# luntergroup/smcsmc

Hardware: AMD Instinct MI355X
Metric: genome segments/sec per EM iteration (Np=10000, 2 diploids, 100 Mb) (higher is better)
Workload: dtype f64

## Files before the change

profiles/stamps.py:

```python
import ctypes as C, os, sys, numpy as np, argparse
ROOT = os.path.dirname(os.path.dirname(os.path.abspath(__file__)))
sys.path.insert(0, ROOT)
from smcsmc_amd import pf, build as _build
ap = argparse.ArgumentParser(); ap.add_argument("--rows", type=int, default=6000); ap.add_argument("--debug", type=int, default=0)
ap.add_argument("--lib", default=None, help="a -DPF_STAMPS library built beforehand (default: build it, smcsmc_amd/build.py)")
a = ap.parse_args()
pf.LIB_PATH = a.lib or _build.build_stamps_lib()
import bench
args = argparse.Namespace(nsam=4, length=1e7, epochs=32, pops=1)
model, segs = bench.build_workload(args, seed=1)
f = pf.ParticleFilter(model, 10000, seed=1, max_trace_events=0, local_recomb=True, debug=a.debug)
f.load_segments(segs)
L = f.L
L.pf_debug_stamps.argtypes = [C.c_void_p, C.c_int64, C.c_void_p]; L.pf_debug_stamps.restype = C.c_int
f.init_prior(0.0); f.run(0, 200); f.sync()
rows = a.rows
assert L.pf_debug_stamps(f.h, rows, None) == 0
f.init_prior(0.0); f.run(0, rows); f.sync()
nc = (10000 + 63) // 64
out = np.zeros((rows, nc, 32), np.uint64)
assert L.pf_debug_stamps(f.h, rows, out.ctypes.data) == 0
st = out[5:, :, :9].astype(np.int64) * 10.0 / 1000.0
flag = f.trace()["resampled"][:rows]
t0 = st[:, :, 0].min(axis=1, keepdims=True)
rel = st - t0[:, :, None]
names = ["start", "loads issued", "decide_row done", "prologue done", "state ready", "update loop done", "site lik done", "stores issued", "scans done"]
end = rel[:, :, 8].max(axis=1)
print("rows", rows, "kernel span (first wave start -> last wave scans done): mean %.2f us" % end.mean())
for sel, nm in ((np.ones(len(end), bool), "all rows"), (flag[4:rows-1] == 1, "rows after a resampling row"), (flag[4:rows-1] == 0, "rows after a plain row")):
    sel = sel[:len(end)]
    print(nm, int(sel.sum()))
    for k in range(9):
        col = rel[sel][:, :, k]
        print("   %-18s mean over waves %6.2f   max over waves (mean over rows) %6.2f" % (names[k], col.mean(), col.max(axis=1).mean()))
    cr = rel[sel]
    idx = cr[:, :, 8].argmax(axis=1)
    crit = cr[np.arange(len(idx)), idx, :]
    print("   critical wave phase durations:", " ".join("%.2f" % v for v in np.diff(crit, axis=1).mean(axis=0)), " start offset %.2f" % crit[:, 0].mean())

sub = out[5:, :, 16:21].astype(np.int64) * 10.0 / 1000.0
selr = (flag[4:rows-1] == 1)[:len(end)]
if selr.any() and sub[selr].max() > 0:
    base = st[selr][:, :, 2]
    seq = [base] + [sub[selr][:, :, k] for k in range(5)] + [st[selr][:, :, 3]]
    nm = ["own offset (pipe_lo_from)", "search over wavefronts", "barrier, range, survivors", "staging decided, barrier", "search inside the wavefront", "first copy?, offspring table, barrier"]
    print("parent search, rows after a resampling row (mean over wavefronts of the step's duration):")
    for k in range(6):
        d = seq[k + 1] - seq[k]
        print("   %-40s %6.2f us" % (nm[k], d.mean()))

d = rel[:, :, 8] - rel[:, :, 4]
m = (len(d) // 2) * 2
pair = (d[0:m:2] + d[1:m:2]).max(axis=1)
single = d[0:m:2].max(axis=1) + d[1:m:2].max(axis=1)
pre = rel[:, :, 4].max(axis=1)
print("own work of a row (state ready -> scans done), slowest wavefront: %.2f us; two rows back to back, slowest wavefront: %.2f us per pair"
      " (two single rows: %.2f us); before it (launch start -> state ready, slowest wavefront): %.2f us" % (d.max(axis=1).mean(), pair.mean(), single.mean(), pre.mean()))
for k in (3, 4):
    mk = (len(d) // k) * k
    grp = sum(d[i:mk:k] for i in range(k)).max(axis=1)
    print("   %d rows back to back: %.2f us per group" % (k, grp.mean()))

acc = out[5:, :, 9:15].astype(np.int64)
trips = acc[:, :, 5].astype(float)
print("update trips per wave and row: mean %.2f, max over waves (mean over rows) %.2f" % (trips.mean(), trips.max(axis=1).mean()))
tot = acc[:, :, :5].sum(axis=(0, 1)) * 10.0 / 1000.0
names2 = ["no-mutation weight (all iterations)", "record head stores", "genealogy update", "record tail + tracked length", "next recombination position"]
for nm, v in zip(names2, tot):
    print("   %-40s %.3f us per trip" % (nm, v / max(1.0, trips.sum())))
acc2 = out[5:, :, 21:29].astype(np.int64)
tot2 = acc2.sum(axis=(0, 1)) * 10.0 / 1000.0
names3 = ["no-mutation weight: up to the factor (fastexp)", "no-mutation weight: the two products, loop control",
          "update: the four draws (table or Philox), next request", "update: cut point (slice, division, lineage)",
          "update: descendant mask", "update: node searches and intensities", "update: walk, inverse search, division",
          "update: tree edit (remove, slots, insert)"]
if tot2.sum() > 0:
    for nm, v in zip(names3, tot2):
        print("      %-52s %.3f us per trip" % (nm, v / max(1.0, trips.sum())))
    print("      %-52s %.3f us per trip" % ("update: tree length (rest of the slot)", (tot[2] - tot2[2:].sum()) / max(1.0, trips.sum())))
st_all = out[5:, :, :9].astype(np.int64) * 10.0 / 1000.0
ci = st_all[:, :, 8].argmax(axis=1)
ct = trips[np.arange(len(ci)), ci]
cl = (st_all[:, :, 5] - st_all[:, :, 4])[np.arange(len(ci)), ci]
print("wavefront that ends the launch: %.2f trips, %.2f us in the loop; wavefront with most trips: %.2f" % (ct.mean(), cl.mean(), trips.max(axis=1).mean()))
```

smcsmc_amd/csrc/pf_hip.hip:

```cpp
#include <hip/hip_runtime.h>
#include <type_traits>
#include <hip/hip_ext.h>

#include <algorithm>
#include <atomic>
#include <cmath>
#include <cstdio>
#include <cstdlib>
#include <cstring>
#include <string>
#include <vector>

#include "../../include/smcsmc_pf.h"
#include "pf_device.h"
#include "pf_types.h"
#include "pf_lane.h"
#include "pf_tree_reg.h"
#include "pf_lds_body.h"
#include "pf_mp_host.h"
#include "pf_wide_host.h"
#include "pf_pipe.h"
#include "pf_lds_pipe.h"

using namespace pf;

__global__ __launch_bounds__(PF_BS) void k_init(KArgs A, double initial_position) {
    extern __shared__ double smem[];
    init_lds_body(A, initial_position, smem);
}

__global__ __launch_bounds__(PF_BS) void k_extend(KArgs A, long long s) {
    extern __shared__ double smem[];
    extend_lds_body(A, s, smem);
}

__device__ __forceinline__ double in_vgpr(double x) { double y; asm("v_mov_b64 %0, %1" : "=v"(y) : "s"(x)); return y; }
__device__ __forceinline__ unsigned long long in_vgpr(unsigned long long x) { unsigned long long y; asm("v_mov_b64 %0, %1" : "=v"(y) : "s"(x)); return y; }

#ifdef PF_STAMPS
__device__ __forceinline__ void pf_acc_trip(unsigned long long* a) { a[5] += 1; }
#else
#define pf_acc_trip(a) do {} while (0)
#endif
#ifdef PF_STAMPS
#define PF_STAMP(k) do { if (A.stamps && (threadIdx.x & 63) == 0 && s < A.stamp_rows)                                   \
        A.stamps[((size_t)s * A.nc + (size_t)(((long long)pf_bx() * PF_BS + threadIdx.x) >> 6)) * PF_STAMP_W + (k)] = wall_clock64(); } while (0)
#define PF_TICK(var) unsigned long long var = wall_clock64()
#define PF_ACC(slot, t0, t1) pf_acc[slot] += (t1) - (t0)
#define PF_ACC_DECL unsigned long long pf_acc[6] = {0, 0, 0, 0, 0, 0}, pf_acc2[8] = {0, 0, 0, 0, 0, 0, 0, 0}
#define PF_ACC2(slot, t0, t1) pf_acc2[slot] += (t1) - (t0)
#define PF_ACC_STORE do { if (A.stamps && (threadIdx.x & 63) == 0 && s < A.stamp_rows) {                                \
        for (int k_ = 0; k_ < 6; ++k_)                                                                                  \
            A.stamps[((size_t)s * A.nc + (size_t)(((long long)pf_bx() * PF_BS + threadIdx.x) >> 6)) * PF_STAMP_W + 9 + k_] = pf_acc[k_]; \
        for (int k_ = 0; k_ < 8; ++k_)                                                                                  \
            A.stamps[((size_t)s * A.nc + (size_t)(((long long)pf_bx() * PF_BS + threadIdx.x) >> 6)) * PF_STAMP_W + 21 + k_] = pf_acc2[k_]; } } while (0)
#else
#define PF_STAMP(k) do {} while (0)
#define PF_TICK(var) do {} while (0)
#define PF_ACC(slot, t0, t1) do {} while (0)
#define PF_ACC2(slot, t0, t1) do {} while (0)
#define PF_ACC_DECL do {} while (0)
#define PF_ACC_STORE do {} while (0)
#endif

template <class KA>
__device__ __forceinline__ int gridDim_particles(const KA& A) { return (int)((A.Np + PF_BS - 1) / PF_BS); }

template <int NM, bool BIASED, bool EXACT = false, bool TREES = false, bool PIPE = false, class KA>
__device__ __forceinline__ void extend_reg_body(const KA& A, long long s, int fuse, PipeRow PR = PipeRow()) {
    extern __shared__ double smem[];
    double* sT = smem;
    double* sH = smem + PF_EPAD;
    double* sI = sH + PF_EPAD;
    double* sBH = sI + A.E;
    double* sBS = sBH + (PF_BIAS_MAX + 2);
    const Ctrl* c = A.ctrl;
    const int n = EXACT ? NM : A.n;
    const long long p = (long long)pf_bx() * PF_BS + threadIdx.x;
    const bool active = p < A.Np;
    const int lane = threadIdx.x & 63;
    PF_STAMP(0);
    RowPre pre;
    RTree<NM> t0;
    double o_wpost = 0.0, o_wpilot = 0.0, o_next = 0.0, o_xmark = 0.0, o_Ltree = 0.0, o_sm = 0.0, o_ebuf = 0.0;
    int o_ml = 0;
    unsigned o_widx = 0;
    unsigned long long o_ctr = 0;
    unsigned o_tab_end = 0;
    long long o_nres = 0; int o_bflag = 0, o_bgen = 0;
    double spec_sm[PF_PIPE_STAGE * 64 / PF_BS];
    int spec_lo = 0;
    double sg_start = 0.0, sg_len = 0.0;
    int sg_limit = 0, sg_state = 1;
    int sg_allele[NM];
#pragma unroll
    for (int i = 0; i < NM; ++i) sg_allele[i] = 0;
    if constexpr (PIPE) {
        if (PR.extend) {
            sg_start = A.seg_start[s]; sg_len = A.seg_len[s];
            sg_limit = A.seg_limit[s]; sg_state = A.seg_state[s];
            const int8_t* al = A.seg_alleles + (size_t)s * n;
#pragma unroll
            for (int i = 0; i < NM; ++i) if (i < n) sg_allele[i] = al[i];
        }
    }
    if constexpr (PIPE) {
        const int fs = __builtin_amdgcn_readfirstlane(PR.slot_prev >= 0 ? PR.slot_prev : c->cur);
        if (PR.complete) {
            pre = row_preload(A, fs);
            o_nres = c->xr[(fs + PF_RING - 1) & (PF_RING - 1)].n_res; o_bflag = c->xr[(fs + PF_RING - 1) & (PF_RING - 1)].flag; o_bgen = c->xr[(fs + PF_RING - 1) & (PF_RING - 1)].gen;
            spec_lo = pf_bx() * (PF_BS / 64) - (PF_PIPE_STAGE - PF_BS / 64) / 2;
            if (spec_lo > A.nc - PF_PIPE_STAGE) spec_lo = A.nc - PF_PIPE_STAGE;
            if (spec_lo < 0) spec_lo = 0;
            if (A.flags & 256) spec_lo = -0x40000000;
            const double* sm0 = A.rg_scan1m + (size_t)fs * A.Np;
#pragma unroll
            for (int k = 0; k < PF_PIPE_STAGE * 64 / PF_BS; ++k) {
                const long long src = (long long)spec_lo * 64 + k * PF_BS + threadIdx.x;
                spec_sm[k] = (src >= 0 && src < A.Np) ? sm0[src] : PF_INF;
            }
        }
        if (active) {
            const DState own = state_slot(A, fs);
#pragma unroll
            for (int r = 0; r < RTree<NM>::NI; ++r) {
                t0.S[r] = 0.0; t0.C0[r] = 0; t0.C1[r] = 0;
                if (r < n - 1) {
                    t0.S[r] = own.S[(size_t)r * A.Np + p];
                    t0.C0[r] = own.C[(size_t)(2 * r) * A.Np + p];
                    t0.C1[r] = own.C[(size_t)(2 * r + 1) * A.Np + p];
                }
            }
            o_wpost = own.w_post[p]; o_wpilot = own.w_pilot[p]; o_next = own.next_base[p]; o_xmark = own.x_mark[p];
            o_ml = own.mark_limit[p]; o_Ltree = own.Ltree[p];
            o_widx = PR.complete ? A.rg_widx[(size_t)fs * A.Np + p] : A.widx[p];
            o_ctr = A.rng_ctr[p]; o_ebuf = A.ebuf[p];
            if (PR.draws) o_tab_end = (unsigned)A.dt_filled[(size_t)((PR.draws - 1) ^ 1) * A.Np + p];
            if (PR.complete) o_sm = A.rg_scan1m[(size_t)fs * A.Np + p];
        }
    }
    for (int e = threadIdx.x; e < PF_EPAD; e += blockDim.x) {
        sT[e] = e < A.E ? A.T[e] : PF_INF;
        sH[e] = e < A.E ? A.Hc[e] : PF_INF;
        if (e < A.E) sI[e] = A.inv2N[e];
    }
    if (BIASED && threadIdx.x < PF_BIAS_MAX + 2) {
        sBH[threadIdx.x] = A.bias_H[threadIdx.x];
        if (threadIdx.x < PF_BIAS_MAX + 1) sBS[threadIdx.x] = A.bias_S[threadIdx.x];
    }
    __shared__ unsigned s_lut[PIPE ? 2 * PF_LUT_N / 4 : 1];
    const bool use_lut = PIPE && A.lut != nullptr;
    if constexpr (PIPE) {
        if (use_lut && threadIdx.x < 2 * PF_LUT_N / 4) s_lut[threadIdx.x] = ((const unsigned*)A.lut)[threadIdx.x];
    }
    int cur = 0, from_slot = 0;
    bool completing = false, gather = false;
    double inv = 1.0, S1v = 0.0, pos_prev = 0.0;
    int lo_p = 0, lo_p1 = 0;
    bool first_copy = true;
    long long a = p;
    int G_end = 0, ev = 0;
    if constexpr (PIPE) {
        PipeLds q = pipe_carve(sBS + (PF_BIAS_MAX + 1), A.nc);
        cur = PR.slot_out; from_slot = PR.slot_prev >= 0 ? PR.slot_prev : c->cur;
        completing = PR.complete != 0;
        pos_prev = PR.pos_prev;
        if (completing) {
            const int row_slot = from_slot;
            const long long n_res = o_nres + o_bflag;
            G_end = o_bgen + o_bflag;
            ev = (int)n_res;
            PF_STAMP(1);
#pragma unroll
            for (int k = 0; k < PF_PIPE_STAGE * 64 / PF_BS; ++k) q.stage[k * PF_BS + threadIdx.x] = spec_sm[k];
            RowDecision d = decide_row<true>(A, q, row_slot, n_res, pre);
            PF_STAMP(2);
            inv = d.inv; S1v = d.S1;
            gather = d.flag != 0;
            if (pf_bx() == 0 && threadIdx.x == 0) {
                Ctrl* cw = A.ctrl;
                cw->xr[row_slot].n_res = n_res; cw->xr[row_slot].gen = G_end; cw->xr[row_slot].flag = d.flag;
            }
            if (gather) {
                const double dn = (double)A.Np;
                const double invS1 = 1.0 / d.S1;
                const double* sm = A.rg_scan1m + (size_t)row_slot * A.Np;
                const int wave = threadIdx.x >> 6;
                int ch_own = (int)(p >> 6);
                double coff_own = 0.0, v_own = 0.0;
                int lo_next = 0;
                if (active) {
                    coff_own = pipe_chunk_offset(q, ch_own);
                    double w = coff_own + o_sm;
                    v_own = q.pmx[ch_own] > w ? q.pmx[ch_own] : w;
                    lo_next = p + 1 < A.Np ? pipe_lo_from(v_own, dn, A.Np, d.S1, invS1, d.u) : (int)A.Np;
                    q.slo[threadIdx.x] = lo_next;
                }
                PF_STAMP(16);
                const double lhs = ((double)p + d.u) * d.S1;
                int pch = 0;
                if (active) {
                    int lo_c = 0, hi_c = A.nc - 1;
                    while (lo_c < hi_c) {
                        int mid = (lo_c + hi_c) >> 1;
                        if (lhs < dn * q.pmx[mid + 1]) hi_c = mid; else lo_c = mid + 1;
                    }
                    pch = lo_c;
                }
                PF_STAMP(17);
                int cmin = active ? pch : 0x7fffffff, cmax = active ? pch : -1;
#pragma unroll
                for (int m = 1; m < 64; m <<= 1) {
                    int o1 = __shfl_xor(cmin, m, 64), o2 = __shfl_xor(cmax, m, 64);
                    cmin = o1 < cmin ? o1 : cmin; cmax = o2 > cmax ? o2 : cmax;
                }
                if (lane == 0) { q.wint[wave] = cmin; q.wint[PF_BS / 64 + wave] = cmax; }
                __syncthreads();
                if (active) lo_p1 = lo_next;
                if (active) {
                    if (threadIdx.x > 0) lo_p = q.slo[threadIdx.x - 1];
                    else lo_p = p > 0 ? pipe_lo_from(q.pmx[ch_own], dn, A.Np, d.S1, invS1, d.u) : 0;
                }
                cmin = q.wint[0]; cmax = q.wint[PF_BS / 64];
                for (int w = 1; w < PF_BS / 64; ++w) {
                    cmin = q.wint[w] < cmin ? q.wint[w] : cmin;
                    cmax = q.wint[PF_BS / 64 + w] > cmax ? q.wint[PF_BS / 64 + w] : cmax;
                }
                {
                    unsigned long long bal = __ballot(active && lo_p1 > lo_p);
                    if (lane == 0) q.wint[2 * (PF_BS / 64) + wave] = __popcll(bal);
                }
                PF_STAMP(18);
                int nst = cmax - cmin + 1;
                if (nst > PF_PIPE_STAGE) nst = PF_PIPE_STAGE;
                if (nst < 0) nst = 0;
                int stage_lo = cmin;
                if (cmin >= spec_lo && cmax < spec_lo + PF_PIPE_STAGE) {
                    stage_lo = spec_lo; nst = PF_PIPE_STAGE;
                } else {
                    __syncthreads();
                    for (int idx = threadIdx.x; idx < nst * 64; idx += PF_BS) {
                        long long src = (long long)cmin * 64 + idx;
                        q.stage[idx] = src < A.Np ? sm[src] : PF_INF;
                    }
                }
                __syncthreads();
                PF_STAMP(19);
                if (threadIdx.x == 0) {
                    int tot = 0;
                    for (int w = 0; w < PF_BS / 64; ++w) tot += q.wint[2 * (PF_BS / 64) + w];
                    A.rg_blkcnt[(size_t)row_slot * gridDim_particles(A) * A.blk_gran + pf_bx()] = tot;
                }
                if (active) {
                    const double coff_p = pipe_chunk_offset(q, pch);
                    const double pm_p = q.pmx[pch];
                    const bool staged = pch >= stage_lo && pch - stage_lo < nst;
                    auto val_at = [&](int l) -> double {
                        long long idx = (long long)pch * 64 + l;
                        double smv = staged ? q.stage[(pch - stage_lo) * 64 + l] : (idx < A.Np ? sm[idx] : PF_INF);
                        double w = coff_p + smv;
                        return pm_p > w ? pm_p : w;
                    };
                    int lo_l = 0, hi_l = 63;
                    while (lo_l < hi_l) {
                        int mid = (lo_l + hi_l) >> 1;
                        if (lhs < dn * val_at(mid)) hi_l = mid; else lo_l = mid + 1;
                    }
                    a = (long long)pch * 64 + lo_l;
                    PF_STAMP(20);
                    if (a > A.Np - 1) a = A.Np - 1;
                    const int la = (int)(a & 63);
                    if (p == 0 || a == 0) first_copy = (p == 0);
                    else {
                        double vprev = la > 0 ? val_at(la - 1) : pm_p;
                        if (a != (long long)pch * 64 + lo_l) {
                            long long am = a - 1;
                            int chm = (int)(am >> 6);
                            double w = pipe_chunk_offset(q, chm) + sm[am];
                            vprev = q.pmx[chm] > w ? q.pmx[chm] : w;
                        }
                        first_copy = ((((double)(p - 1)) + d.u) * d.S1 < dn * vprev);
                    }
                    int* lo_tab = A.lo + (size_t)(G_end % A.Gcap) * (A.Np + 1);
                    lo_tab[p] = lo_p;
                    if (p == A.Np - 1) lo_tab[A.Np] = (int)A.Np;
                }
            }
        }
    } else {
        cur = c->cur;
        completing = fuse != 0;
        gather = fuse && c->flag;
        from_slot = gather ? (cur ^ 1) : cur;
        __syncthreads();
    }
    if constexpr (PIPE) __syncthreads();
    PF_STAMP(3);
    cur = __builtin_amdgcn_readfirstlane(cur);
    from_slot = __builtin_amdgcn_readfirstlane(from_slot);
    double w_post = 0.0, w_pilot = 0.0;
    bool has_pending = false;
    if (active) {
        const DState st = state_slot(A, cur);
        const DState from = state_slot(A, from_slot);
        if constexpr (!PIPE) {
            a = gather ? (long long)A.parent[p] : p;
            const int* lo_tab = A.lo + (size_t)((c->gen - 1 + A.Gcap) % A.Gcap) * (A.Np + 1);
            if (gather) { lo_p = lo_tab[p]; lo_p1 = lo_tab[p + 1]; first_copy = (p == lo_tab[a]); }
            inv = c->inv_T; S1v = c->S1; pos_prev = c->cur_pos;
            G_end = c->gen - 1; ev = (int)c->n_resample - 1;
        }
        RTree<NM> t;
        const bool reload = !PIPE || gather;
        if (!reload) t = t0;
        else {
#pragma unroll
            for (int r = 0; r < RTree<NM>::NI; ++r) {
                t.S[r] = 0.0; t.C0[r] = 0; t.C1[r] = 0;
                if (r < n - 1) {
                    t.S[r] = from.S[(size_t)r * A.Np + a];
                    t.C0[r] = from.C[(size_t)(2 * r) * A.Np + a];
                    t.C1[r] = from.C[(size_t)(2 * r + 1) * A.Np + a];
                }
            }
        }
        RCtx cx;
        const double v_L = in_vgpr(A.L), v_mu = in_vgpr(A.mu), v_rho = in_vgpr(A.rho);
        cx.T = sT; cx.I = sI; cx.H = sH; cx.E = A.E; cx.n = n; cx.L = v_L; cx.mu = v_mu; cx.rho = v_rho;
        cx.seed = in_vgpr(A.seed); cx.slot = (unsigned)p; cx.stream = 0;
        cx.nb = A.n_bias + 1; cx.bH = sBH; cx.bS = sBS; cx.last_iw = 1.0;
        cx.want_desc = A.lmap_opp != nullptr || TREES; cx.want_desc_new = TREES; cx.last_desc = 0; cx.last_desc_new = 0;
        cx.vbc = A.vb_coal; cx.upd_fac = 1.0;
        cx.gK = BIASED ? A.g_K : 0; cx.gpos = A.g_pos; cx.grho = A.g_rho; cx.gleaf = A.g_leaf; cx.last_rbiw = 1.0;
        cx.ridx = cx.gK > 0 ? from.ridx[a] : 0; cx.g_rp = 0; cx.g_sb = 0;
        if constexpr (PIPE) {
            cx.lutT = use_lut ? (const unsigned char*)s_lut : nullptr;
            cx.lutH = use_lut ? (const unsigned char*)s_lut + PF_LUT_N : nullptr;
            cx.kbT = A.lut_kbT; cx.kbH = A.lut_kbH;
            cx.tab = nullptr; cx.tab_end = 0; cx.pf_ok = false; cx.pf_ctr = 0; cx.draws_log = false;
            if (PR.draws) {
                cx.tab = (const double2*)A.dt_tab + (size_t)p * PF_DRAW_RING;
                cx.tab_end = o_tab_end;
            }
        }
        DStore ds;
        if (BIASED) {
            d_bind(ds, A, st, p);
            ds.count = from.dcount[a]; ds.total = from.total_delayed[a];
            if (gather || PIPE)
                for (int k = 0; k < ds.count; ++k) {
                    st.dpos[(size_t)k * A.Np + p] = from.dpos[(size_t)k * A.Np + a];
                    st.dfac[(size_t)k * A.Np + p] = from.dfac[(size_t)k * A.Np + a];
                    st.ddelta[(size_t)k * A.Np + p] = from.ddelta[(size_t)k * A.Np + a];
                    st.dk[(size_t)k * A.Np + p] = from.dk[(size_t)k * A.Np + a];
                }
        }
        double next_base, x_mark;
        int mark_limit;
        unsigned widx;
        if (reload) {
            w_post = from.w_post[a];
            w_pilot = from.w_pilot[a];
            next_base = from.next_base[a];
            x_mark = from.x_mark[a];
            mark_limit = from.mark_limit[a];
            cx.Ltree = from.Ltree[a];
        } else {
            w_post = o_wpost; w_pilot = o_wpilot; next_base = o_next; x_mark = o_xmark; mark_limit = o_ml; cx.Ltree = o_Ltree;
        }
        if constexpr (PIPE) { cx.ctr = o_ctr; cx.ebuf = o_ebuf; widx = o_widx; r_draws_prefetch(cx); }
        else { cx.ctr = A.rng_ctr[p]; cx.ebuf = A.ebuf[p]; widx = A.widx[p]; }
        if (completing) {
            if (!PIPE && p == 0) { Ctrl* cw = A.ctrl; cw->gen_prev = c->gen; cw->nres_prev = c->n_resample; }
            if (!gather) {
                w_post *= inv;
                w_pilot *= inv;
            } else {
                const int G = G_end;
                const double pos = pos_prev;
                const DState& src = from;
                if (lo_p1 > lo_p) {
                    double* rec = rec_ptr(A, p, widx);
                    rec[0] = PIPE ? o_xmark : src.x_mark[p];
                    rec[1] = pos;
                    rec[2] = 0.0; rec[3] = 0.0;
                    rec[4] = __longlong_as_double((long long)make_meta(1, PIPE ? o_ml : src.mark_limit[p], -1, n));
                    if constexpr (PIPE) {
#pragma unroll
                        for (int r = 0; r < RTree<NM>::NI; ++r) if (r < n - 1) rec[5 + r] = t0.S[r];
                    } else {
                        for (int r = 0; r < n - 1; ++r) rec[5 + r] = src.S[(size_t)r * A.Np + p];
                    }
                    ++widx;
                }
                A.gstart[(size_t)((G + 1) % A.Gcap) * A.Np + p] = widx;
                if (ev < A.max_trace_events) A.ev_parents[(size_t)ev * A.Np + p] = (int)a;
                double wp = w_post * inv;
                double wq = w_pilot * inv;
                double sumn = S1v * inv;
                double adj = sumn / ((double)A.Np * wq);
                w_post = wp * adj;
                w_pilot = wq * adj;
                x_mark = pos;
                if (!first_copy && pos < v_L) {
                    next_base = r_sample_next_base<false>(cx, pos);
                    if constexpr (PIPE) r_draws_prefetch(cx);
                }
            }
        }

        PF_STAMP(4);
        const bool do_extend = !PIPE || PR.extend != 0;
        const int8_t* data = A.seg_alleles + (size_t)s * n;
        double seg_end = 0.0;
        int limit = 0;
        if constexpr (PIPE) { if (do_extend) { seg_end = sg_start + sg_len; limit = sg_limit; } }
        else { if (do_extend) { seg_end = A.seg_start[s] + A.seg_len[s]; limit = A.seg_limit[s]; } }
        const double extend_to = seg_end < v_L ? seg_end : v_L;
        unsigned one_mask = 0, zero_mask = 0, present_mask = 0, two_mask = 0;
        int missing = 0;
        if (do_extend)
#pragma unroll
            for (int i = 0; i < NM; ++i) if (i < n) {
                int d = PIPE ? sg_allele[i] : (int)data[i];
                missing += d == -1;
                if (d == 1) one_mask |= 1u << i;
                if (d == 0) zero_mask |= 1u << i;
                if (d == 2) two_mask |= 1u << i;
                if (d >= 0) present_mask |= 1u << i;
            }
        int leaf_status = 0;
        if (missing == 0) leaf_status = 1;
        if (missing == n) leaf_status = -1;

        double updated_to = (PIPE && completing) ? pos_prev : c->cur_pos;
        if (!do_extend) updated_to = extend_to;
        double B;
        if (leaf_status == -1) B = 0;
        else if (leaf_status == 1) B = cx.Ltree;
        else B = r_tracked_len(t, n, present_mask);

        PF_ACC_DECL;
        while (updated_to < extend_to) {
            PF_TICK(tk0);
            double new_to = extend_to < next_base ? extend_to : next_base;
            double f = fastexp(-v_mu * B * (new_to - updated_to));
            PF_TICK(tk0a);
            PF_ACC2(0, tk0, tk0a);
            w_post *= f;
            w_pilot *= f;
            if (BIASED && cx.gK > 0) {
                double dist = new_to - updated_to;
                double target_rate = dist * v_rho * cx.Ltree;
                double sampled_rate = dist * cx.grho[cx.ridx] * cx.Ltree;
                double iws = fastexp(sampled_rate - target_rate);
                w_post *= iws;
                w_pilot *= iws;
            }
            updated_to = new_to;
            if (BIASED && cx.gK > 0 && updated_to < extend_to && cx.ridx + 1 < cx.gK && updated_to == cx.gpos[cx.ridx + 1]) {
                cx.ridx += 1;
                next_base = r_sample_next_base<false>(cx, updated_to);
                if constexpr (PIPE) r_draws_prefetch(cx);
                continue;
            }
            PF_TICK(tk1);
            PF_ACC(0, tk0, tk1);
            PF_ACC2(1, tk0a, tk1);
            if (updated_to < extend_to) {
                double* rec = rec_ptr(A, p, widx);
                rec[0] = x_mark;
                rec[1] = updated_to;
#pragma unroll
                for (int r = 0; r < RTree<NM>::NI; ++r) if (r < n - 1) rec[5 + r] = t.S[r];
                double h, tc;
                PF_TICK(tk2);
                PF_ACC(1, tk1, tk2);
                r_genealogy_update<NM, BIASED, PIPE, PIPE && EXACT && NM == 4 && !BIASED && !TREES>(cx, t, &h, &tc);
                PF_TICK(tk3);
                PF_ACC(2, tk2, tk3);
#ifdef PF_STAMPS
                PF_ACC2(2, tk2, cx.gt[0]);
                for (int k_ = 0; k_ < 5; ++k_) PF_ACC2(3 + k_, cx.gt[k_], cx.gt[k_ + 1]);
#endif
                if (cx.vbc) { w_post *= cx.upd_fac; w_pilot *= cx.upd_fac; cx.upd_fac = 1.0; }
                rec[2] = h;
                rec[3] = tc;
                rec[4] = __longlong_as_double((long long)make_meta(0, mark_limit, limit, n, cx.last_desc, TREES ? cx.last_desc_new : 0u));
                ++widx;
                if (leaf_status == 0) B = r_tracked_len(t, n, present_mask);
                if (leaf_status == 1) B = cx.Ltree;
                PF_TICK(tk4);
                PF_ACC(3, tk3, tk4);
                pf_acc_trip(pf_acc);
                if (BIASED) {
                    double iw = cx.last_iw, rbiw = cx.last_rbiw;
                    double delay_height = (A.delay_type & 3) == 0 ? h : tc;
                    int idx = 0;
                    while (idx + 1 < cx.nb + 1 && sBH[idx + 1] < delay_height) ++idx;
                    if (idx >= cx.nb) idx = cx.nb - 1;
                    if (sBS[idx] == 1.0 && !(A.delay_type & 4)) { w_post *= rbiw; w_pilot *= rbiw; iw /= rbiw; }
                    double delay = A.app_delays[r_epoch_of(cx, delay_height)];
                    d_adjust_with_delay(ds, w_post, w_pilot, iw, delay, updated_to);
                }
                PF_TICK(tk5);
                next_base = r_sample_next_base<true, PIPE>(cx, updated_to);
                x_mark = updated_to;
                mark_limit = limit;
                PF_TICK(tk6);
                PF_ACC(4, tk5, tk6);
            }
        }
        PF_ACC_STORE;

        PF_STAMP(5);
        const KA& A1 = pf_reopen(A);
        const DState st1 = state_slot(A1, cur);
        if (BIASED) {
            for (;;) {
                if (ds.count == 0 || !do_extend) break;
                double pm = ds.pos[0];
                for (int i = 1; i < ds.count; ++i) { double pi = ds.pos[(size_t)i * ds.Np]; if (pi < pm) pm = pi; }
                if (!(pm < extend_to)) break;
                d_apply_earliest(ds, w_pilot);
            }
            st1.dcount[p] = ds.count;
            st1.total_delayed[p] = ds.total;
            if (cx.gK > 0) st1.ridx[p] = cx.ridx;
            has_pending = ds.count > 0;
        }
        if (do_extend && (PIPE ? sg_state : (int)A1.seg_state[s]) == 0) {
            const bool dephase = A1.flags & 2;
            const bool anc = A1.flags & 1;
            unsigned het_pairs = 0;
            int ncfg = 1;
            for (int i = 0; i + 1 < n; i += 2) {
                bool d0_two = (two_mask >> i) & 1u;
                bool one0 = (one_mask >> i) & 1u, one1 = (one_mask >> (i + 1)) & 1u;
                bool zero0 = (zero_mask >> i) & 1u, zero1 = (zero_mask >> (i + 1)) & 1u;
                bool het = d0_two || (dephase && ((one0 && zero1) || (zero0 && one1)));
                if (het) {
                    ncfg *= 2;
                    het_pairs |= 1u << i;
                    one_mask &= ~(3u << i); zero_mask &= ~(3u << i);
                    zero_mask |= 1u << i;
                    one_mask |= 1u << (i + 1);
                }
            }
            double norm = 1.0 / (double)ncfg;
            RBranchP<NM> bprob;
            r_site_branch_probs(t, n, v_mu, bprob);
            double lik = 0;
            for (;;) {
                lik += r_site_lik_from(t, n, bprob, one_mask, zero_mask, anc);
                if (ncfg == 1) break;
                bool more = false;
                for (int i = 0; i + 1 < n; i += 2) {
                    if (!((het_pairs >> i) & 1)) continue;
                    if ((zero_mask >> i) & 1) {
                        zero_mask &= ~(1u << i); one_mask |= 1u << i;
                        one_mask &= ~(1u << (i + 1)); zero_mask |= 1u << (i + 1);
                        more = true;
                        break;
                    }
                    one_mask &= ~(1u << i); zero_mask |= 1u << i;
                    zero_mask &= ~(1u << (i + 1)); one_mask |= 1u << (i + 1);
                }
                if (!more) break;
            }
            lik *= norm;
            w_post *= lik;
            w_pilot *= lik;
        }

        PF_STAMP(6);
#pragma unroll
        for (int r = 0; r < RTree<NM>::NI; ++r)
            if (r < n - 1) {
                st1.S[(size_t)r * A1.Np + p] = t.S[r];
                st1.C[(size_t)(2 * r) * A1.Np + p] = (int8_t)t.C0[r];
                st1.C[(size_t)(2 * r + 1) * A1.Np + p] = (int8_t)t.C1[r];
            }
        st1.w_post[p] = w_post;
        st1.w_pilot[p] = w_pilot;
        st1.next_base[p] = next_base;
        st1.x_mark[p] = x_mark;
        st1.mark_limit[p] = mark_limit;
        st1.Ltree[p] = cx.Ltree;
        A1.rng_ctr[p] = cx.ctr;
        A1.ebuf[p] = cx.ebuf;
        if constexpr (PIPE) {
            if (PR.draws) A1.dt_ctr[(size_t)(PR.draws - 1) * A1.Np + p] = cx.ctr;
            A1.rg_widx[(size_t)cur * A1.Np + p] = widx;
            if (!do_extend) A1.widx[p] = widx;
            if (PR.ahead) {
                const unsigned kold = A1.gstart[(size_t)(A1.ctrl->g_safe % A1.Gcap) * A1.Np + p];
                if (widx - kold > A1.cap && !A1.ctrl->err) A1.ctrl->err = ERR_LOG_OVERFLOW;
            }
        } else {
            A1.widx[p] = widx;
        }
        if (TREES && widx >= A1.cap) A1.ctrl->err = ERR_LOG_OVERFLOW;
        if constexpr (!PIPE) {
#pragma unroll
            for (int r = 0; r < RTree<NM>::NI; ++r) if (r < n - 1) A1.snap_S[A1.sp][(size_t)r * A1.Np + p] = t.S[r];
            A1.snap_w[A1.sp][p] = w_post; A1.snap_xm[A1.sp][p] = x_mark; A1.snap_ml[A1.sp][p] = mark_limit; A1.snap_widx[A1.sp][p] = widx;
        }
    }
    PF_STAMP(7);
    const KA& A2 = pf_reopen(A);
    double sp = wave_tree_sum(w_post);
    double sq = wave_tree_sum(w_pilot * w_pilot);
    double sc = wave_hs_scan(w_pilot, lane);
    double scp = wave_hs_scan(w_post, lane);
    double scm = wave_max_scan_d(sc, lane);
    long long chunk = p >> 6;
    PF_STAMP(8);
    if constexpr (PIPE) {
        const size_t ro = (size_t)cur * A2.Np, co = (size_t)cur * A2.nc;
        if (active) { A2.rg_scan1[ro + p] = sc; A2.rg_scanp[ro + p] = scp; A2.rg_scan1m[ro + p] = scm; }
        if (p == A2.Np - 1) A2.ctrl->last1[cur] = sc;
        if (lane == 63 && chunk < A2.nc) {
            A2.rg_cpost[co + chunk] = sp;
            A2.rg_csq[co + chunk] = sq;
            A2.rg_cpil[co + chunk] = sc;
            A2.rg_cpp[co + chunk] = scp;
            A2.rg_cmx1[co + chunk] = scm;
        }
        if (BIASED) {
            unsigned long long pend = __ballot(has_pending);
            if (lane == 0 && chunk < A2.nc) {
                A2.rg_dpend[co + chunk] = __popcll(pend);
                if (!PR.extend) A2.chunk_dpend[chunk] = __popcll(pend);
            }
        }
    } else {
        if (active) { A2.scan1[p] = sc; A2.scanp2[A2.sp][p] = scp; A2.scan1m[p] = scm; }
        if (lane == 63 && chunk < (A2.Np + 63) / 64) {
            A2.chunk_post[chunk] = sp;
            A2.chunk_sq[chunk] = sq;
            A2.chunk_pil[chunk] = sc;
            A2.chunk_pp[chunk] = scp;
            A2.chunk_mx1[chunk] = scm;
        }
        if (BIASED) {
            unsigned long long pend = __ballot(has_pending);
            if (lane == 0 && chunk < (A2.Np + 63) / 64) A2.chunk_dpend[chunk] = __popcll(pend);
        }
    }
}

template <int NM, bool BIASED, bool TREES = false>
__global__ __launch_bounds__(PF_BS) void k_extend_reg(KArgs A, long long s, int fuse) {
    extend_reg_body<NM, BIASED, false, TREES>(A, s, fuse);
}

#define PF_FIN_TILE_B 64
#define PF_FIN_PAIRS 64

template <class KA>
__device__ void finalize_counts(const KA& A, Ctrl* c, int tid, int nthreads, double* stage ) {
    const int E = A.E;
    const int nb = A.nbx;
// ... 3770 lines not shown
```

Baseline: 40210.

## Issue parent state loads early in resampling prologue, drop cross-wave staging

After: 40280, median of 4. No clear change (+0.2%).

```diff
diff --git a/profiles/stamps.py b/profiles/stamps.py
--- a/profiles/stamps.py
+++ b/profiles/stamps.py
@@ -43,11 +43,14 @@
 if selr.any() and sub[selr].max() > 0:
     base = st[selr][:, :, 2]
     seq = [base] + [sub[selr][:, :, k] for k in range(5)] + [st[selr][:, :, 3]]
-    nm = ["own offset (pipe_lo_from)", "search over wavefronts", "barrier, range, survivors", "staging decided, barrier", "search inside the wavefront", "first copy?, offspring table, barrier"]
-    print("parent search, rows after a resampling row (mean over wavefronts of the step's duration):")
+    nm = ["search over wavefronts", "search inside the wavefront", "parent's state requested, own offset (pipe_lo_from)",
+          "barrier, offsets exchanged, survivors", "first copy?, offspring table", "barrier, survivor sum"]
+    print("prologue, rows after a resampling row (mean over wavefronts of the step's duration):")
     for k in range(6):
         d = seq[k + 1] - seq[k]
-        print("   %-40s %6.2f us" % (nm[k], d.mean()))
+        print("   %-52s %6.2f us" % (nm[k], d.mean()))
+    far = out[5:, :, 29].astype(np.int64)[selr]
+    print("   lanes that read the scans from memory: %.3f %% of the lanes of these rows (%d rows with any)" % (100.0 * far.sum() / (selr.sum() * 10000.0), int((far.sum(axis=1) > 0).sum())))
 
 d = rel[:, :, 8] - rel[:, :, 4]
 m = (len(d) // 2) * 2
diff --git a/smcsmc_amd/csrc/pf_hip.hip b/smcsmc_amd/csrc/pf_hip.hip
--- a/smcsmc_amd/csrc/pf_hip.hip
+++ b/smcsmc_amd/csrc/pf_hip.hip
@@ -36,6 +36,12 @@
 
 __device__ __forceinline__ double in_vgpr(double x) { double y; asm("v_mov_b64 %0, %1" : "=v"(y) : "s"(x)); return y; }
 __device__ __forceinline__ unsigned long long in_vgpr(unsigned long long x) { unsigned long long y; asm("v_mov_b64 %0, %1" : "=v"(y) : "s"(x)); return y; }
+
+__device__ __forceinline__ void pf_lds_barrier() {
+    __builtin_amdgcn_fence(__ATOMIC_RELEASE, "workgroup", "local");
+    __builtin_amdgcn_s_barrier();
+    __builtin_amdgcn_fence(__ATOMIC_ACQUIRE, "workgroup", "local");
+}
 
 #ifdef PF_STAMPS
 __device__ __forceinline__ void pf_acc_trip(unsigned long long* a) { a[5] += 1; }
@@ -160,6 +166,9 @@
     bool first_copy = true;
     long long a = p;
     int G_end = 0, ev = 0;
+    RTree<NM> tpar;
+    double pa_wpost = 0.0, pa_wpilot = 0.0, pa_next = 0.0, pa_xmark = 0.0, pa_Ltree = 0.0, pa_total = 0.0;
+    int pa_ml = 0, pa_ridx = 0, pa_dcount = 0;
     if constexpr (PIPE) {
         PipeLds q = pipe_carve(sBS + (PF_BIAS_MAX + 1), A.nc);
         cur = PR.slot_out; from_slot = PR.slot_prev >= 0 ? PR.slot_prev : c->cur;
@@ -186,17 +195,6 @@
                 const double invS1 = 1.0 / d.S1;
                 const double* sm = A.rg_scan1m + (size_t)row_slot * A.Np;
                 const int wave = threadIdx.x >> 6;
-                int ch_own = (int)(p >> 6);
-                double coff_own = 0.0, v_own = 0.0;
-                int lo_next = 0;
-                if (active) {
-                    coff_own = pipe_chunk_offset(q, ch_own);
-                    double w = coff_own + o_sm;
-                    v_own = q.pmx[ch_own] > w ? q.pmx[ch_own] : w;
-                    lo_next = p + 1 < A.Np ? pipe_lo_from(v_own, dn, A.Np, d.S1, invS1, d.u) : (int)A.Np;
-                    q.slo[threadIdx.x] = lo_next;
-                }
-                PF_STAMP(16);
                 const double lhs = ((double)p + d.u) * d.S1;
                 int pch = 0;
                 if (active) {
@@ -207,68 +205,75 @@
                     }
                     pch = lo_c;
                 }
+                PF_STAMP(16);
+                const double coff_p = pipe_chunk_offset(q, pch);
+                const double pm_p = q.pmx[pch];
+                const bool staged = pch >= spec_lo && pch - spec_lo < PF_PIPE_STAGE;
+                auto val_at = [&](int l) -> double {
+                    long long idx = (long long)pch * 64 + l;
+                    double smv = q.stage[(staged ? (pch - spec_lo) * 64 : 0) + l];
+                    if (!staged) { smv = idx < A.Np ? sm[idx] : PF_INF; asm volatile("" : "+v"(smv)); }
+                    double w = coff_p + smv;
+                    return pm_p > w ? pm_p : w;
+                };
+                int lo_l = 0;
+                if (active) {
+                    int hi_l = 63;
+                    while (lo_l < hi_l) {
+                        int mid = (lo_l + hi_l) >> 1;
+                        if (lhs < dn * val_at(mid)) hi_l = mid; else lo_l = mid + 1;
+                    }
+                    a = (long long)pch * 64 + lo_l;
+                    if (a > A.Np - 1) a = A.Np - 1;
+                }
                 PF_STAMP(17);
-                int cmin = active ? pch : 0x7fffffff, cmax = active ? pch : -1;
+#ifdef PF_STAMPS
+                {
+                    const unsigned long long far = __ballot(active && !staged);
+                    if (A.stamps && lane == 0 && s < A.stamp_rows)
+                        A.stamps[((size_t)s * A.nc + (size_t)(((long long)pf_bx() * PF_BS + threadIdx.x) >> 6)) * PF_STAMP_W + 29] = __popcll(far);
+                }
+#endif
+                if (active) {
+                    const DState from = state_slot(A, __builtin_amdgcn_readfirstlane(row_slot));
 #pragma unroll
-                for (int m = 1; m < 64; m <<= 1) {
-                    int o1 = __shfl_xor(cmin, m, 64), o2 = __shfl_xor(cmax, m, 64);
-                    cmin = o1 < cmin ? o1 : cmin; cmax = o2 > cmax ? o2 : cmax;
+                    for (int r = 0; r < RTree<NM>::NI; ++r) {
+                        tpar.S[r] = 0.0; tpar.C0[r] = 0; tpar.C1[r] = 0;
+                        if (r < n - 1) {
+                            tpar.S[r] = from.S[(size_t)r * A.Np + a];
+                            tpar.C0[r] = from.C[(size_t)(2 * r) * A.Np + a];
+                            tpar.C1[r] = from.C[(size_t)(2 * r + 1) * A.Np + a];
+                        }
+                    }
+                    pa_wpost = from.w_post[a]; pa_wpilot = from.w_pilot[a]; pa_next = from.next_base[a]; pa_xmark = from.x_mark[a];
+                    pa_ml = from.mark_limit[a]; pa_Ltree = from.Ltree[a];
+                    if (BIASED) {
+                        if (A.g_K > 0) pa_ridx = from.ridx[a];
+                        pa_dcount = from.dcount[a]; pa_total = from.total_delayed[a];
+                    }
                 }
-                if (lane == 0) { q.wint[wave] = cmin; q.wint[PF_BS / 64 + wave] = cmax; }
-                __syncthreads();
+                const int ch_own = (int)(p >> 6);
+                int lo_next = 0;
+                if (active) {
+                    const double coff_own = pipe_chunk_offset(q, ch_own);
+                    double w = coff_own + o_sm;
+                    const double v_own = q.pmx[ch_own] > w ? q.pmx[ch_own] : w;
+                    lo_next = p + 1 < A.Np ? pipe_lo_from(v_own, dn, A.Np, d.S1, invS1, d.u) : (int)A.Np;
+                    q.slo[threadIdx.x] = lo_next;
+                }
+                PF_STAMP(18);
+                pf_lds_barrier();
                 if (active) lo_p1 = lo_next;
                 if (active) {
                     if (threadIdx.x > 0) lo_p = q.slo[threadIdx.x - 1];
                     else lo_p = p > 0 ? pipe_lo_from(q.pmx[ch_own], dn, A.Np, d.S1, invS1, d.u) : 0;
                 }
-                cmin = q.wint[0]; cmax = q.wint[PF_BS / 64];
-                for (int w = 1; w < PF_BS / 64; ++w) {
-                    cmin = q.wint[w] < cmin ? q.wint[w] : cmin;
-                    cmax = q.wint[PF_BS / 64 + w] > cmax ? q.wint[PF_BS / 64 + w] : cmax;
-                }
                 {
                     unsigned long long bal = __ballot(active && lo_p1 > lo_p);
-                    if (lane == 0) q.wint[2 * (PF_BS / 64) + wave] = __popcll(bal);
+                    if (lane == 0) q.wint[wave] = __popcll(bal);
                 }
-                PF_STAMP(18);
-                int nst = cmax - cmin + 1;
-                if (nst > PF_PIPE_STAGE) nst = PF_PIPE_STAGE;
-                if (nst < 0) nst = 0;
-                int stage_lo = cmin;
-                if (cmin >= spec_lo && cmax < spec_lo + PF_PIPE_STAGE) {
-                    stage_lo = spec_lo; nst = PF_PIPE_STAGE;
-                } else {
-                    __syncthreads();
-                    for (int idx = threadIdx.x; idx < nst * 64; idx += PF_BS) {
-                        long long src = (long long)cmin * 64 + idx;
-                        q.stage[idx] = src < A.Np ? sm[src] : PF_INF;
-                    }
-                }
-                __syncthreads();
                 PF_STAMP(19);
-                if (threadIdx.x == 0) {
-                    int tot = 0;
-                    for (int w = 0; w < PF_BS / 64; ++w) tot += q.wint[2 * (PF_BS / 64) + w];
-                    A.rg_blkcnt[(size_t)row_slot * gridDim_particles(A) * A.blk_gran + pf_bx()] = tot;
-                }
                 if (active) {
-                    const double coff_p = pipe_chunk_offset(q, pch);
-                    const double pm_p = q.pmx[pch];
-                    const bool staged = pch >= stage_lo && pch - stage_lo < nst;
-                    auto val_at = [&](int l) -> double {
-                        long long idx = (long long)pch * 64 + l;
-                        double smv = staged ? q.stage[(pch - stage_lo) * 64 + l] : (idx < A.Np ? sm[idx] : PF_INF);
-                        double w = coff_p + smv;
-                        return pm_p > w ? pm_p : w;
-                    };
-                    int lo_l = 0, hi_l = 63;
-                    while (lo_l < hi_l) {
-                        int mid = (lo_l + hi_l) >> 1;
-                        if (lhs < dn * val_at(mid)) hi_l = mid; else lo_l = mid + 1;
-                    }
-                    a = (long long)pch * 64 + lo_l;
-                    PF_STAMP(20);
-                    if (a > A.Np - 1) a = A.Np - 1;
                     const int la = (int)(a & 63);
                     if (p == 0 || a == 0) first_copy = (p == 0);
                     else {
@@ -285,6 +290,7 @@
                     lo_tab[p] = lo_p;
                     if (p == A.Np - 1) lo_tab[A.Np] = (int)A.Np;
                 }
+                PF_STAMP(20);
             }
         }
     } else {
@@ -294,7 +300,15 @@
         from_slot = gather ? (cur ^ 1) : cur;
         __syncthreads();
     }
-    if constexpr (PIPE) __syncthreads();
+    if constexpr (PIPE) {
+        pf_lds_barrier();
+        if (gather && threadIdx.x == 0) {
+            PipeLds q = pipe_carve(sBS + (PF_BIAS_MAX + 1), A.nc);
+            int tot = 0;
+            for (int w = 0; w < PF_BS / 64; ++w) tot += q.wint[w];
+            A.rg_blkcnt[(size_t)from_slot * gridDim_particles(A) * A.blk_gran + pf_bx()] = tot;
+        }
+    }
     PF_STAMP(3);
     cur = __builtin_amdgcn_readfirstlane(cur);
     from_slot = __builtin_amdgcn_readfirstlane(from_slot);
@@ -313,6 +327,7 @@
         RTree<NM> t;
         const bool reload = !PIPE || gather;
         if (!reload) t = t0;
+        else if (PIPE) t = tpar;
         else {
 #pragma unroll
             for (int r = 0; r < RTree<NM>::NI; ++r) {
@@ -332,7 +347,7 @@
         cx.want_desc = A.lmap_opp != nullptr || TREES; cx.want_desc_new = TREES; cx.last_desc = 0; cx.last_desc_new = 0;
         cx.vbc = A.vb_coal; cx.upd_fac = 1.0;
         cx.gK = BIASED ? A.g_K : 0; cx.gpos = A.g_pos; cx.grho = A.g_rho; cx.gleaf = A.g_leaf; cx.last_rbiw = 1.0;
-        cx.ridx = cx.gK > 0 ? from.ridx[a] : 0; cx.g_rp = 0; cx.g_sb = 0;
+        cx.ridx = cx.gK > 0 ? (PIPE && gather ? pa_ridx : from.ridx[a]) : 0; cx.g_rp = 0; cx.g_sb = 0;
         if constexpr (PIPE) {
             cx.lutT = use_lut ? (const unsigned char*)s_lut : nullptr;
             cx.lutH = use_lut ? (const unsigned char*)s_lut + PF_LUT_N : nullptr;
@@ -346,7 +361,8 @@
         DStore ds;
         if (BIASED) {
             d_bind(ds, A, st, p);
-            ds.count = from.dcount[a]; ds.total = from.total_delayed[a];
+            if (PIPE && gather) { ds.count = pa_dcount; ds.total = pa_total; }
+            else { ds.count = from.dcount[a]; ds.total = from.total_delayed[a]; }
             if (gather || PIPE)
                 for (int k = 0; k < ds.count; ++k) {
                     st.dpos[(size_t)k * A.Np + p] = from.dpos[(size_t)k * A.Np + a];
@@ -358,7 +374,9 @@
         double next_base, x_mark;
         int mark_limit;
         unsigned widx;
-        if (reload) {
+        if (PIPE && reload) {
+            w_post = pa_wpost; w_pilot = pa_wpilot; next_base = pa_next; x_mark = pa_xmark; mark_limit = pa_ml; cx.Ltree = pa_Ltree;
+        } else if (reload) {
             w_post = from.w_post[a];
             w_pilot = from.w_pilot[a];
             next_base = from.next_base[a];
```
